# SakodaShintaro/f2-nerf

Measured on AMD Instinct MI355X. Metric: rendered rays/sec (fwd+bwd) at 800x800, higher is better.
Workload: dtype f32; 1 GPU; ngp_fox-like synthetic views 800x800, 128 samples/ray, L=16 F=2 T=2^19, 65536-ray chunks, TRAIN render + loss + backward (optimizer excluded); pixel_order=rows, regime=dense

## Files before the change

f2-nerf_amd/csrc/kernels/hash_grid.hip:

```cpp
#include "hash_grid.hiph"


namespace
{


__global__ __launch_bounds__(F2N_BLOCK) void table_to_f16_kernel(
  const float * __restrict__ in, uint16_t * __restrict__ out, int64_t n)
{
  const int64_t stride = (int64_t)gridDim.x * blockDim.x * 8;
  for (int64_t i = ((int64_t)blockIdx.x * blockDim.x + threadIdx.x) * 8; i < n; i += stride) {
    if (i + 8 <= n) {
      const float4 a = *reinterpret_cast<const float4 *>(in + i);
      const float4 b = *reinterpret_cast<const float4 *>(in + i + 4);
      uint4 o;
      o.x = (uint32_t)__half_as_ushort(__float2half_rn(a.x)) |
            ((uint32_t)__half_as_ushort(__float2half_rn(a.y)) << 16);
      o.y = (uint32_t)__half_as_ushort(__float2half_rn(a.z)) |
            ((uint32_t)__half_as_ushort(__float2half_rn(a.w)) << 16);
      o.z = (uint32_t)__half_as_ushort(__float2half_rn(b.x)) |
            ((uint32_t)__half_as_ushort(__float2half_rn(b.y)) << 16);
      o.w = (uint32_t)__half_as_ushort(__float2half_rn(b.z)) |
            ((uint32_t)__half_as_ushort(__float2half_rn(b.w)) << 16);
      *reinterpret_cast<uint4 *>(out + i) = o;
    } else {
      for (int64_t j = i; j < n; j++) out[j] = __half_as_ushort(__float2half_rn(in[j]));
    }
  }
}


template <int F, bool POW2>
__global__ __launch_bounds__(F2N_BLOCK) void hash_fwd_kernel(
  const float * __restrict__ pts, const uint16_t * __restrict__ table,
  const int32_t * __restrict__ primes, const float * __restrict__ bias,
  const float * __restrict__ mul, float * __restrict__ out, int64_t out_ld_point,
  int64_t out_ld_chan, uint32_t * __restrict__ idx_out, int64_t n, int L, uint32_t T,
  int64_t level_stride)
{
  const int l = blockIdx.y;
  const int64_t p = (int64_t)blockIdx.x * F2N_BLOCK + threadIdx.x;
  if (p >= n) return;
  const LevelParams lp = load_level(primes, bias, mul, l);
  const float x = pts[3 * p + 0], y = pts[3 * p + 1], z = pts[3 * p + 2];
  uint32_t row[8];
  float w[8];
  corner_rows_and_weights<POW2>(x, y, z, lp, T, row, w);
  float acc[F];
  gather_blend<F>(table + level_stride * l, row, w, acc);
  float * o = out + p * out_ld_point + (int64_t)(l * F) * out_ld_chan;
#pragma unroll
  for (int k = 0; k < F; k++) o[k * out_ld_chan] = round_f16(acc[k]);
  if (idx_out) {
    uint32_t * io = idx_out + (p * L + l) * 8;
#pragma unroll
    for (int d = 0; d < 8; d++) io[d] = row[d];
  }
}


template <int F, bool POW2, int SAMPLES>
__global__ __launch_bounds__(F2N_BLOCK) void hash_fwd_raytile_kernel(
  const float * __restrict__ pts, const uint16_t * __restrict__ table,
  const int32_t * __restrict__ primes, const float * __restrict__ bias,
  const float * __restrict__ mul, float * __restrict__ out, int n_rays, int S, uint32_t T,
  int64_t level_stride, int walk, int corner_order)
{
  static_assert(F2N_BLOCK == 256 && SAMPLES % 16 == 0, "4 waves, float4 runs");
  constexpr int RAYS = 64, kPitch = SAMPLES + 4, kPPitch = 3 * SAMPLES + 1;
  __shared__ __attribute__((aligned(16))) float tile[F][RAYS][kPitch];
  __shared__ float ptile[RAYS][kPPitch];
  const int l = blockIdx.y;
  const int tiles_s = S / SAMPLES;
  const int r0 = (int)(blockIdx.x / tiles_s) * RAYS, k0 = (int)(blockIdx.x % tiles_s) * SAMPLES;
  const int lane = threadIdx.x & 63, wave = threadIdx.x >> 6;
  const int64_t n = (int64_t)n_rays * S;
#pragma unroll
  for (int i = 0; i < RAYS * 3 * SAMPLES / 256; i++) {
    const int idx = threadIdx.x + 256 * i;
    const int ray = idx / (3 * SAMPLES), off = idx % (3 * SAMPLES);
    const int r = min(r0 + ray, n_rays - 1);
    ptile[ray][off] = pts[((int64_t)r * S + k0) * 3 + off];
  }
  const LevelParams lp = load_level(primes, bias, mul, l);
  __syncthreads();
  bool along, drifted;
  {
    constexpr int m = SAMPLES / 2;
    auto dist = [&](int ra, int sa, int rb, int sb) {
      const float dx = ptile[ra][3 * sa] - ptile[rb][3 * sb], dy = ptile[ra][3 * sa + 1] - ptile[rb][3 * sb + 1],
                  dz = ptile[ra][3 * sa + 2] - ptile[rb][3 * sb + 2];
      return sqrtf(dx * dx + dy * dy + dz * dz);
    };
    const float e = dist(RAYS - 1, m, 0, m), e1 = dist(1, m, 0, m), sl = dist(0, SAMPLES - 1, 0, 0);
    along = !(e + 8.f * e1 < 2.f * sl);
    if (walk) along = (walk == 2);
    const float apart = fmaxf(e1, fmaxf(dist(RAYS / 2 + 1, m, RAYS / 2, m), dist(RAYS - 1, m, RAYS - 2, m)));
    drifted = apart * (float)(SAMPLES - 1) > 0.35f * sl;
  }
  __shared__ uint16_t order[RAYS * SAMPLES];
  __shared__ uint32_t bin_at[64];
  const bool sorted = !along && (walk == 3 || (walk == 0 && drifted));
  if (sorted) {
    constexpr int kPairs = RAYS * SAMPLES / 256;
    constexpr int mr = RAYS / 2;
    const float ax = ptile[mr][3 * (SAMPLES - 1)] - ptile[mr][0],
                ay = ptile[mr][3 * (SAMPLES - 1) + 1] - ptile[mr][1],
                az = ptile[mr][3 * (SAMPLES - 1) + 2] - ptile[mr][2];
    const float inv = 64.f / fmaxf(ax * ax + ay * ay + az * az, 1e-30f);
    const float ox = ptile[mr][0], oy = ptile[mr][1], oz = ptile[mr][2];
    if (threadIdx.x < 64) bin_at[threadIdx.x] = 0u;
    __syncthreads();
    int my_bin[kPairs];
#pragma unroll
    for (int i = 0; i < kPairs; i++) {
      const int pair = threadIdx.x + 256 * i, ray = pair / SAMPLES, ks = pair % SAMPLES;
      const float d = (ptile[ray][3 * ks] - ox) * ax + (ptile[ray][3 * ks + 1] - oy) * ay +
                      (ptile[ray][3 * ks + 2] - oz) * az;
      my_bin[i] = min(max((int)(d * inv), 0), 63);
      atomicAdd(&bin_at[my_bin[i]], 1u);
    }
    __syncthreads();
    if (wave == 0) {
      const int c = (int)bin_at[lane];
      bin_at[lane] = (uint32_t)(wave_incl_scan_i32(c) - c);
    }
    __syncthreads();
#pragma unroll
    for (int i = 0; i < kPairs; i++)
      order[atomicAdd(&bin_at[my_bin[i]], 1u)] = (uint16_t)(threadIdx.x + 256 * i);
    __syncthreads();
  }
  constexpr int kRaysPerIter = 64 / SAMPLES;
  auto walk_tile = [&](auto paired) {
#pragma unroll
    for (int j = 0; j < SAMPLES / 4; j++) {
      int ks = along ? (lane % SAMPLES) : (j * 4 + wave);
      int ray = along ? ((j * 4 + wave) * kRaysPerIter + lane / SAMPLES) : lane;
      if (sorted) {
        const int pair = order[(j * 4 + wave) * 64 + lane];
        ray = pair / SAMPLES;
        ks = pair % SAMPLES;
      }
      const float x = ptile[ray][3 * ks], y = ptile[ray][3 * ks + 1], z = ptile[ray][3 * ks + 2];
      uint32_t row[8];
      float w[8], acc[F];
      if constexpr (decltype(paired)::value) {
        const uint32_t m = slot_rows_and_weights<POW2>(x, y, z, lp, T, row, w);
        gather_blend_paired<F>(table + level_stride * l, row, m, w, acc);
      } else {
        corner_rows_and_weights<POW2>(x, y, z, lp, T, row, w);
        gather_blend<F>(table + level_stride * l, row, w, acc);
      }
#pragma unroll
      for (int k = 0; k < F; k++) tile[k][ray][ks] = round_f16(acc[k]);
    }
  };
  if (corner_order == 0)
    walk_tile(std::true_type{});
  else
    walk_tile(std::false_type{});
  __syncthreads();
#pragma unroll
  for (int i = 0; i < SAMPLES / 16; i++) {
    const int idx = threadIdx.x + 256 * i;
    const int ray = idx / (SAMPLES / 4), quad = idx % (SAMPLES / 4);
    if (r0 + ray < n_rays) {
#pragma unroll
      for (int k = 0; k < F; k++) {
        const float4 v = *reinterpret_cast<const float4 *>(&tile[k][ray][4 * quad]);
        *reinterpret_cast<float4 *>(
          out + (int64_t)(l * F + k) * n + (int64_t)(r0 + ray) * S + k0 + 4 * quad) = v;
      }
    }
  }
}


template <int F, bool POW2, bool WITH_PTS_GRAD>
__global__ __launch_bounds__(F2N_BLOCK) void hash_bwd_kernel(
  const float * __restrict__ pts, const uint16_t * __restrict__ table,
  const int32_t * __restrict__ primes, const float * __restrict__ bias,
  const float * __restrict__ mul, const float * __restrict__ grad_out, int64_t g_ld_point,
  int64_t g_ld_chan, float * __restrict__ table_grad, float * __restrict__ pts_grad, int64_t n,
  uint32_t T, int64_t level_stride, float grad_scale, float inv_scale)
{
  const int l = blockIdx.y;
  const int64_t p = (int64_t)blockIdx.x * F2N_BLOCK + threadIdx.x;
  if (p >= n) return;
  const LevelParams lp = load_level(primes, bias, mul, l);
  const float x = pts[3 * p + 0], y = pts[3 * p + 1], z = pts[3 * p + 2];
  uint32_t row[8];
  float w[8];
  corner_rows_and_weights<POW2>(x, y, z, lp, T, row, w);

  const float * g = grad_out + p * g_ld_point + (int64_t)(l * F) * g_ld_chan;
  float gk[F];
  bool any = false;
#pragma unroll
  for (int k = 0; k < F; k++) {
    gk[k] = round_f16(g[k * g_ld_chan] * grad_scale);
    any |= (gk[k] != 0.f);
  }
  float * gbase = table_grad + level_stride * l;
  if (any) {
#pragma unroll
    for (int d = 0; d < 8; d++) {
#pragma unroll
      for (int k = 0; k < F; k++) {
        const float c = round_f16(gk[k] * w[d]) * inv_scale;
        atomicAdd(gbase + (int64_t)row[d] * F + k, c);
      }
    }
  }
  if (WITH_PTS_GRAD) {
    using Row = typename RowBits<F>::type;
    const Row * rows = reinterpret_cast<const Row *>(table + level_stride * l);
    float gx = 0.f, gy = 0.f, gz = 0.f;
#pragma unroll
    for (int d = 0; d < 8; d++) {
      float f[F];
      const Row r = rows[row[d]];
      unpack_row<F>(r, f);
#pragma unroll
      for (int k = 0; k < F; k++) {
        const float nrm = f[k] * lp.mul * gk[k];
        const float pos = round_f16(nrm), neg = round_f16(-nrm);
        gx += (d & 4) ? pos : neg;
        gy += (d & 2) ? pos : neg;
        gz += (d & 1) ? pos : neg;
      }
    }
    atomicAdd(pts_grad + 3 * p + 0, gx * inv_scale);
    atomicAdd(pts_grad + 3 * p + 1, gy * inv_scale);
    atomicAdd(pts_grad + 3 * p + 2, gz * inv_scale);
  }
}

constexpr int kSliceFloats = 32768;
constexpr int kSliceBlock = 1024;

template <int F, bool POW2>
__global__ __launch_bounds__(kSliceBlock) void hash_bwd_sliced_kernel(
  const float * __restrict__ pts, const int32_t * __restrict__ primes,
  const float * __restrict__ bias, const float * __restrict__ mul,
  const float * __restrict__ grad_out, int64_t g_ld_point, int64_t g_ld_chan,
  float * __restrict__ table_grad, int64_t n, uint32_t T, int64_t level_stride, float grad_scale,
  float inv_scale, int n_parts)
{
  __shared__ float acc[kSliceFloats];
  constexpr uint32_t kRows = kSliceFloats / F;
  const uint32_t slice = blockIdx.x;
  const int l = blockIdx.y;
  const int part = blockIdx.z;
  const uint32_t row_lo = slice * kRows;

  for (int i = threadIdx.x; i < kSliceFloats; i += kSliceBlock) acc[i] = 0.f;
  __syncthreads();

  const LevelParams lp = load_level(primes, bias, mul, l);
  const int64_t per = (n + n_parts - 1) / n_parts;
  const int64_t p_begin = per * part;
  const int64_t p_end = (p_begin + per < n) ? p_begin + per : n;
  const float * gcol = grad_out + (int64_t)(l * F) * g_ld_chan;

  struct Item
  {
    float x, y, z;
    float g[F];
  };
  auto fetch = [&](int64_t p, Item & it) {
    it.x = pts[3 * p + 0];
    it.y = pts[3 * p + 1];
    it.z = pts[3 * p + 2];
    const float * g = gcol + p * g_ld_point;
#pragma unroll
    for (int k = 0; k < F; k++) it.g[k] = g[k * g_ld_chan];
  };
  auto apply = [&](const Item & it) {
    uint32_t row[8];
    float w[8];
    corner_rows_and_weights<POW2>(it.x, it.y, it.z, lp, T, row, w);
    float gk[F];
#pragma unroll
    for (int k = 0; k < F; k++) gk[k] = round_f16(it.g[k] * grad_scale);
#pragma unroll
    for (int d = 0; d < 8; d++) {
      const uint32_t local = row[d] - row_lo;
      if (local < kRows) {
#pragma unroll
        for (int k = 0; k < F; k++) {
          const float c = round_f16(gk[k] * w[d]);
          if (c != 0.f) atomicAdd(&acc[local * F + k], c);
        }
      }
    }
  };

  int64_t p = p_begin + threadIdx.x;
  if (p < p_end) {
    Item cur, nxt;
    fetch(p, cur);
    for (; p < p_end; p += kSliceBlock) {
      const int64_t pn = (p + kSliceBlock < p_end) ? p + kSliceBlock : p;
      fetch(pn, nxt);
      apply(cur);
      cur = nxt;
    }
  }
  __syncthreads();

  float * gbase = table_grad + level_stride * l + (int64_t)row_lo * F;
  const uint32_t rows_here = (row_lo + kRows <= T) ? kRows : (T > row_lo ? T - row_lo : 0u);
  const int n_flush = (int)rows_here * F;
  for (int i = threadIdx.x; i < n_flush; i += kSliceBlock) {
    const float v = acc[i];
    if (v != 0.f) atomicAdd(gbase + i, v * inv_scale);
  }
}


__global__ __launch_bounds__(F2N_BLOCK) void contract_fwd_kernel(
  const float * __restrict__ pts, float * __restrict__ out, int64_t n)
{
  const int64_t p = (int64_t)blockIdx.x * F2N_BLOCK + threadIdx.x;
  if (p >= n) return;
  float x = pts[3 * p], y = pts[3 * p + 1], z = pts[3 * p + 2];
  contract_point(x, y, z);
  out[3 * p] = x;
  out[3 * p + 1] = y;
  out[3 * p + 2] = z;
}

__global__ __launch_bounds__(F2N_BLOCK) void contract_bwd_kernel(
  const float * __restrict__ pts, const float * __restrict__ dx, float * __restrict__ dp, int64_t n)
{
  const int64_t p = (int64_t)blockIdx.x * F2N_BLOCK + threadIdx.x;
  if (p >= n) return;
  const float x = pts[3 * p], y = pts[3 * p + 1], z = pts[3 * p + 2];
  const float gx = dx[3 * p], gy = dx[3 * p + 1], gz = dx[3 * p + 2];
  const float n2 = fmaf(z, z, fmaf(y, y, x * x));
  const float nrm = sqrtf(n2);
  float ox, oy, oz;
  if (nrm <= 1.f) {
    const float poison = (nrm == 0.f) ? __builtin_nanf("") : 0.f;
    ox = gx + poison;
    oy = gy + poison;
    oz = gz + poison;
  } else {
    const float inv = 1.f / nrm;
    const float a = (2.f - inv) * inv;
    const float da_over_n = (2.f * inv - 2.f) * inv * inv * inv;
    const float pg = fmaf(z, gz, fmaf(y, gy, x * gx));
    const float c = da_over_n * pg;
    ox = fmaf(c, x, a * gx);
    oy = fmaf(c, y, a * gy);
    oz = fmaf(c, z, a * gz);
  }
  dp[3 * p] = ox;
  dp[3 * p + 1] = oy;
  dp[3 * p + 2] = oz;
}

}

extern "C" int f2n_table_to_f16(
  const float * table_f32, uint16_t * table_f16, int64_t n, void * stream)
{
  if (!table_f32 || !table_f16 || n < 0) return F2N_E_INVALID_ARG;
  if (n == 0) return F2N_OK;
  if ((reinterpret_cast<uintptr_t>(table_f32) & 15u) || (reinterpret_cast<uintptr_t>(table_f16) & 15u))
    return F2N_E_INVALID_ARG;
  const int64_t work = (n + 7) / 8;
  const unsigned grid = (unsigned)std::min<int64_t>((work + F2N_BLOCK - 1) / F2N_BLOCK, 256 * 16);
  hipLaunchKernelGGL(
    table_to_f16_kernel, dim3(grid), dim3(F2N_BLOCK), 0, (hipStream_t)stream, table_f32, table_f16,
    n);
  return f2n_launch_status();
}

extern "C" int f2n_hash_fwd(
  const float * pts, const uint16_t * table_f16, const int32_t * primes, const float * bias,
  const float * mul, float * out, int64_t out_ld_point, int64_t out_ld_chan, uint32_t * idx_out,
  int64_t n, int L, int F, uint32_t T, int64_t level_stride, void * stream)
{
  if (!pts || !table_f16 || !primes || !bias || !mul || !out) return F2N_E_INVALID_ARG;
  if (F != 1 && F != 2 && F != 4 && F != 8) return F2N_E_UNSUPPORTED;
  if (!f2n_hash_args_ok(n, L, F, T, level_stride)) return F2N_E_INVALID_ARG;
  if (reinterpret_cast<uintptr_t>(table_f16) % (2u * F)) return F2N_E_INVALID_ARG;
  if (n == 0) return F2N_OK;
  const dim3 grid(f2n_div_up(n, F2N_BLOCK), (unsigned)L), block(F2N_BLOCK);
  hipStream_t s = (hipStream_t)stream;
  f2n_dispatch_field(F, T, [&](auto ff, auto p2) {
    hipLaunchKernelGGL(
      (hash_fwd_kernel<decltype(ff)::value, decltype(p2)::value>), grid, block, 0, s, pts,
      table_f16, primes, bias, mul, out, out_ld_point, out_ld_chan, idx_out, n, L, T, level_stride);
  });
  return f2n_launch_status();
}

extern "C" int f2n_hash_fwd_raytile(
  const float * pts, const uint16_t * table_f16, const int32_t * primes, const float * bias,
  const float * mul, float * out_cm, int n_rays, int S, int L, int F, uint32_t T,
  int64_t level_stride, void * stream)
{
  if (!pts || !table_f16 || !primes || !bias || !mul || !out_cm) return F2N_E_INVALID_ARG;
  if (F != 1 && F != 2 && F != 4 && F != 8) return F2N_E_UNSUPPORTED;
  if (n_rays < 0 || S <= 0) return F2N_E_INVALID_ARG;
  if (S % 16) return F2N_E_UNSUPPORTED;
  const int64_t n = (int64_t)n_rays * S;
  if (!f2n_hash_args_ok(n, L, F, T, level_stride)) return F2N_E_INVALID_ARG;
  if (reinterpret_cast<uintptr_t>(table_f16) % (2u * F)) return F2N_E_INVALID_ARG;
  if (reinterpret_cast<uintptr_t>(out_cm) & 15u) return F2N_E_INVALID_ARG;
  if (n == 0) return F2N_OK;
  const int walk = f2n_get_option(F2N_OPT_RAYTILE_WALK);
  const int corner_order = f2n_get_option(F2N_OPT_GATHER_PAIRED);
  const int want = f2n_get_option(F2N_OPT_RAYTILE);
  const int ts = (want == 16) ? 16 : (S % 32 == 0 ? 32 : 16);
  const int64_t tiles = (int64_t)f2n_div_up(n_rays, 64) * (S / ts);
  if (tiles > 0x7fffffff) return F2N_E_INVALID_ARG;
  const dim3 grid((unsigned)tiles, (unsigned)L), block(F2N_BLOCK);
  hipStream_t s = (hipStream_t)stream;
  f2n_dispatch_field(F, T, [&](auto ff, auto p2) {
    constexpr int FF = decltype(ff)::value;
    constexpr bool P2 = decltype(p2)::value;
    if (ts == 16)
      hipLaunchKernelGGL(
        (hash_fwd_raytile_kernel<FF, P2, 16>), grid, block, 0, s, pts, table_f16, primes, bias, mul,
        out_cm, n_rays, S, T, level_stride, walk, corner_order);
    else
      hipLaunchKernelGGL(
        (hash_fwd_raytile_kernel<FF, P2, 32>), grid, block, 0, s, pts, table_f16, primes, bias, mul,
        out_cm, n_rays, S, T, level_stride, walk, corner_order);
  });
  return f2n_launch_status();
}

extern "C" int f2n_hash_bwd(
  const float * pts, const uint16_t * table_f16, const int32_t * primes, const float * bias,
  const float * mul, const float * grad_out, int64_t g_ld_point, int64_t g_ld_chan,
  float * table_grad, float * pts_grad, int64_t n, int L, int F, uint32_t T, int64_t level_stride,
  float grad_scale, void * stream)
{
  if (!pts || !table_f16 || !primes || !bias || !mul || !grad_out || !table_grad)
    return F2N_E_INVALID_ARG;
  if (F != 1 && F != 2 && F != 4 && F != 8) return F2N_E_UNSUPPORTED;
  if (!f2n_hash_args_ok(n, L, F, T, level_stride)) return F2N_E_INVALID_ARG;
  if (reinterpret_cast<uintptr_t>(table_f16) % (2u * F)) return F2N_E_INVALID_ARG;
  int e = 0;
  const float m = frexpf(grad_scale, &e);
  if (!(grad_scale > 0.f) || m != 0.5f) return F2N_E_INVALID_ARG;
  if (n == 0) return F2N_OK;
  hipStream_t s = (hipStream_t)stream;
  const float inv = 1.f / grad_scale;

  const int64_t rows_per_slice = kSliceFloats / F;
  const int64_t n_slices = ((int64_t)T + rows_per_slice - 1) / rows_per_slice;
  const int force = f2n_get_option(F2N_OPT_HASH_BWD);
  bool sliced = !pts_grad && n_slices <= 64 && n >= 32768;
  if (force && !pts_grad && n_slices <= 1024) sliced = (force == 2);
  if (sliced) {
    int n_parts = 1;
    while ((int64_t)L * n_slices * n_parts < 512 && (n / (n_parts * 2)) >= 65536) n_parts *= 2;
    const dim3 grid((unsigned)n_slices, (unsigned)L, (unsigned)n_parts), block(kSliceBlock);
    f2n_dispatch_field(F, T, [&](auto ff, auto p2) {
      hipLaunchKernelGGL(
        (hash_bwd_sliced_kernel<decltype(ff)::value, decltype(p2)::value>), grid, block, 0, s, pts,
        primes, bias, mul, grad_out, g_ld_point, g_ld_chan, table_grad, n, T, level_stride,
        grad_scale, inv, n_parts);
    });
    return f2n_launch_status();
  }

  if (pts_grad) {
    if (hipMemsetAsync(pts_grad, 0, sizeof(float) * 3 * n, s) != hipSuccess) return F2N_E_LAUNCH;
  }
  const dim3 grid(f2n_div_up(n, F2N_BLOCK), (unsigned)L), block(F2N_BLOCK);
  f2n_dispatch_field(F, T, [&](auto ff, auto p2) {
    constexpr int FF = decltype(ff)::value;
    constexpr bool P2 = decltype(p2)::value;
    if (pts_grad)
      hipLaunchKernelGGL(
        (hash_bwd_kernel<FF, P2, true>), grid, block, 0, s, pts, table_f16, primes, bias, mul,
        grad_out, g_ld_point, g_ld_chan, table_grad, pts_grad, n, T, level_stride, grad_scale, inv);
    else
      hipLaunchKernelGGL(
        (hash_bwd_kernel<FF, P2, false>), grid, block, 0, s, pts, table_f16, primes, bias, mul,
        grad_out, g_ld_point, g_ld_chan, table_grad, pts_grad, n, T, level_stride, grad_scale, inv);
  });
  return f2n_launch_status();
}

extern "C" int f2n_contract_fwd(const float * pts, float * x, int64_t n, void * stream)
{
  if (!pts || !x || n < 0) return F2N_E_INVALID_ARG;
  if (n == 0) return F2N_OK;
  hipLaunchKernelGGL(
    contract_fwd_kernel, dim3(f2n_div_up(n, F2N_BLOCK)), dim3(F2N_BLOCK), 0, (hipStream_t)stream,
    pts, x, n);
  return f2n_launch_status();
}

extern "C" int f2n_contract_bwd(
  const float * pts, const float * dx, float * dpts, int64_t n, void * stream)
{
  if (!pts || !dx || !dpts || n < 0) return F2N_E_INVALID_ARG;
  if (n == 0) return F2N_OK;
  hipLaunchKernelGGL(
    contract_bwd_kernel, dim3(f2n_div_up(n, F2N_BLOCK)), dim3(F2N_BLOCK), 0, (hipStream_t)stream,
    pts, dx, dpts, n);
  return f2n_launch_status();
}
```

include/f2nerf_hip.h:

```cpp
#ifndef F2NERF_HIP_H_
#define F2NERF_HIP_H_

#include <stdint.h>

#ifdef __cplusplus
extern "C" {
#endif

#define F2N_ABI_VERSION 2

#define F2N_OK 0
#define F2N_E_INVALID_ARG (-1)
#define F2N_E_LAUNCH (-2)
#define F2N_E_UNSUPPORTED (-3)

#define F2N_MAX_LEVELS 32

int f2n_abi_version(void);
const char * f2n_status_string(int status);

#define F2N_OPT_SHADE_FWD 0
#define F2N_OPT_SHADE_BWD 1
#define F2N_OPT_SHADE_VARIANT 2
#define F2N_OPT_RAYTILE 3
#define F2N_OPT_HASH_BWD 4
#define F2N_OPT_BWD_COMBINE 5
#define F2N_OPT_RAYTILE_WALK 6
#define F2N_OPT_MARCH 7
#define F2N_OPT_BWD_PHASES 8
#define F2N_OPT_RAY_ORDER 9
#define F2N_OPT_SHADE_BWD_WAVES 10
#define F2N_SHADE_BWD_TWO_WAVES_MIN_SAMPLES (3 << 19)
#define F2N_OPT_SHADE_RAYS 11
#define F2N_OPT_DENSE_LEAN 12
#define F2N_OPT_COUNT 13
#define F2N_OPT2_FIRST 64
#define F2N_OPT_GATHER_PAIRED (F2N_OPT2_FIRST + 0)
#define F2N_OPT2_COUNT 1
int f2n_set_option(int key, int value);
int f2n_get_option(int key);


int f2n_table_to_f16(const float * table_f32, uint16_t * table_f16, int64_t n, void * stream);

int f2n_hash_fwd(
  const float * pts, const uint16_t * table_f16, const int32_t * primes, const float * bias,
  const float * mul, float * out, int64_t out_ld_point, int64_t out_ld_chan, uint32_t * idx_out,
  int64_t n, int L, int F, uint32_t T, int64_t level_stride, void * stream);

int f2n_hash_fwd_raytile(
  const float * pts, const uint16_t * table_f16, const int32_t * primes, const float * bias,
  const float * mul, float * out_cm, int n_rays, int S, int L, int F, uint32_t T,
  int64_t level_stride, void * stream);

int f2n_hash_bwd(
  const float * pts, const uint16_t * table_f16, const int32_t * primes, const float * bias,
  const float * mul, const float * grad_out, int64_t g_ld_point, int64_t g_ld_chan,
  float * table_grad, float * pts_grad, int64_t n, int L, int F, uint32_t T, int64_t level_stride,
  float grad_scale, void * stream);

int64_t f2n_hash_bwd_workspace_bytes(int64_t n, int L, int F, uint32_t T);
int f2n_hash_bwd_set_overflow_counter(uint64_t * device_counter);
int f2n_hash_bwd_binned(
  const float * pts, const int32_t * primes, const float * bias, const float * mul,
  const float * grad_out, int64_t g_ld_point, int64_t g_ld_chan, float * table_grad, int64_t n,
  int L, int F, uint32_t T, int64_t level_stride, float grad_scale, void * workspace,
  int64_t workspace_bytes, void * stream);

int f2n_contract_fwd(const float * pts, float * x, int64_t n, void * stream);
int f2n_contract_bwd(const float * pts, const float * dx, float * dpts, int64_t n, void * stream);

int f2n_hash_rays_grad(
  const float * pts, const float * t, const int32_t * bounds, const float * rays_d,
  const uint16_t * table_f16, const int32_t * primes, const float * bias, const float * mul,
  const float * grad_out, int64_t g_ld_point, int64_t g_ld_chan, float * d_rays_o,
  float * d_rays_d, int n_rays, int L, int F, uint32_t T, int64_t level_stride, float grad_scale,
  void * stream);


int f2n_sh_encode(const float * dirs, float * out, int64_t n, int degree, void * stream);


int f2n_seg_sum_fwd(const float * val, const int32_t * idx, float * sum, int n_rays, void * stream);
int f2n_seg_sum_bwd(const float * dsum, const int32_t * idx, float * dval, int n_rays, void * stream);
int f2n_seg_sum_vec_fwd(
  const float * val, const int32_t * idx, float * sum, int n_rays, int vec, void * stream);
int f2n_seg_sum_vec_bwd(
  const float * dsum, const int32_t * idx, float * dval, int n_rays, int vec, void * stream);
int f2n_seg_scan_fwd(
  const float * val, const int32_t * idx, float * sum, int n_rays, int include_this, void * stream);
int f2n_seg_scan_bwd(
  const float * dsum, const int32_t * idx, float * dval, int n_rays, int include_this,
  void * stream);

int f2n_weight_var_fwd(
  const float * weights, const int32_t * idx, float * out_vars, int n_rays, void * stream);
int f2n_weight_var_bwd(
  const float * weights, const int32_t * idx, const float * dvars, float * dw, int n_rays,
  void * stream);

int f2n_weight_dist_fwd(
  const float * weights, const float * t, const float * dt, const int32_t * idx, float * out,
  int n_rays, void * stream);
int f2n_weight_dist_bwd(
  const float * weights, const float * t, const float * dt, const int32_t * idx,
  const float * d_out, float * dw, int n_rays, void * stream);


int f2n_scatter_idx(
  const int32_t * idx, const int32_t * emb_idx, int32_t * all_emb_idx, int n_rays, void * stream);
int f2n_scatter_add_fwd(
  const float * emb, const int32_t * scatter_idx, const float * to_add, float * sum, int64_t n_all,
  int C, void * stream);
int f2n_scatter_add_bwd(
  const int32_t * scatter_idx, const float * dsum, float * demb, int64_t n_all, int n_emb, int C,
  void * stream);


int f2n_gen_rays(
  const float * poses, int pose_ld, const float * intrinsics, int64_t n_cams,
  const int32_t * cam_idx, const int32_t * ij, int64_t first_pixel, int width, float * rays_o,
  float * rays_d, int64_t n, void * stream);

int64_t f2n_gen_rays_bwd_workspace_floats(int64_t n);
int f2n_gen_rays_bwd(
  const float * intrinsics, int64_t n_cams, const int32_t * ij, int64_t first_pixel, int width,
  const float * d_rays_o, const float * d_rays_d, float * d_poses, int pose_ld, float * workspace,
  int64_t n, void * stream);

int f2n_gen_rays_dist(
  const float * poses, int pose_ld, const float * intrinsics, const float * dist, int64_t n_cams,
  const int32_t * cam_idx, const int32_t * ij, int64_t first_pixel, int width, float * rays_o,
  float * rays_d, int64_t n, void * stream);

int f2n_gen_rays_dist_bwd(
  const float * intrinsics, const float * dist, int64_t n_cams, const int32_t * ij,
  int64_t first_pixel, int width, const float * d_rays_o, const float * d_rays_d, float * d_poses,
  int pose_ld, float * workspace, int64_t n, void * stream);

int64_t f2n_cam_pose_grad_workspace_floats(int64_t n, int64_t n_cams);
int f2n_cam_pose_grad(
  const float * intrinsics, const float * dist, const int32_t * ij, const float * d_rays_o,
  const float * d_rays_d, const int32_t * cam_start, const int32_t * order, float * d_poses,
  int pose_ld, float * workspace, int64_t n, int64_t n_cams, void * stream);

int f2n_pose_compose(
  const float * base, int pose_ld, const float * delta, const int32_t * fixed, float * out,
  int64_t n_cams, void * stream);

int f2n_pose_compose_bwd(
  const float * base, int pose_ld, const float * delta, const int32_t * fixed, const float * d_out,
  float * d_delta, int64_t n_cams, void * stream);

int f2n_project_points(
  const float * points, const float * poses, int pose_ld, const float * intrinsics,
  const float * dist, int64_t n_cams, const int32_t * cam_idx, float * pix, int32_t * valid,
  int64_t n, void * stream);

int f2n_sample_rays(
  const float * rays_o, const float * rays_d, const float * noise, float * pts, float * dirs,
  float * dt, float * t, int32_t * bounds, int n_rays, int S, float step, void * stream);

int f2n_sample_dense(
  const float * rays_o, const float * rays_d, const float * noise, const int32_t * noise_row,
  int noise_affine, float * x, float * dt, float * t, int32_t * bounds, float * ray_dirs,
  int n_rays, int S, float step, void * stream);

int f2n_density_march(
  const float * rays_o, const float * rays_d, const float * noise, const uint16_t * table_f16,
  const int32_t * primes, const float * bias, const float * mul, const float * w0, const float * b0,
  int32_t * kept, int n_rays, int S, float step, int L, int F, uint32_t T, int64_t level_stride,
  float t_thresh, float density_shift, void * stream);

int f2n_density_scan(
  const float * enc_cm, int C, const float * dt, const float * w0, const float * b0, int32_t * kept,
  int n_rays, int S, float t_thresh, float density_shift, void * stream);

int f2n_density_margin(
  const float * logit, const float * dt, int32_t * flag, int n_rays, int S, float density_shift,
  float depth_limit, void * stream);

int f2n_compact_rows_cm(
  const float * src, int64_t n_src, float * dst, int64_t n_dst, int C, const int32_t * bounds,
  int n_rays, int S, void * stream);

int f2n_bounds_from_counts(
  const int32_t * kept, int32_t * bounds, int32_t * total, int n_rays, void * stream);

int f2n_sample_compact(
  const float * rays_o, const float * rays_d, const float * noise, const int32_t * bounds,
  float * pts, float * dirs, float * dt, float * t, int n_rays, int S, float step, void * stream);



int f2n_occ_update(
  const uint16_t * table_f16, const int32_t * primes, const float * bias, const float * mul,
  const float * w0, const float * b0, const float * probe_u, float * density, uint32_t * bits, int G,
  int L, int F, uint32_t T, int64_t level_stride, float density_shift, float threshold, float decay,
  void * stream);

int f2n_occ_lookup(
  const float * pts, int64_t n, const uint32_t * bits, int G, uint8_t * out, void * stream);

int f2n_density_march_occ(
  const float * rays_o, const float * rays_d, const float * noise, const uint16_t * table_f16,
  const int32_t * primes, const float * bias, const float * mul, const float * w0, const float * b0,
  const uint32_t * bits, int G, int32_t * kept, int32_t * len, int n_rays, int S, float step, int L,
  int F, uint32_t T, int64_t level_stride, float t_thresh, float density_shift, void * stream);

int f2n_sample_compact_occ(
  const float * rays_o, const float * rays_d, const float * noise, const int32_t * bounds,
  const int32_t * len, const uint32_t * bits, int G, float * pts, float * dirs, float * dt,
  float * t, int n_rays, int S, float step, void * stream);


int f2n_ray_keys(const float * rays_d, int32_t * keys, int n, void * stream);

int f2n_ray_permute(
  const int64_t * order, int n, int S, const float * rays_o, const float * rays_d,
  const int32_t * emb_idx, const float * bg, const float * noise, int32_t * perm, float * rays_o_p,
  float * rays_d_p, int32_t * emb_idx_p, float * bg_p, float * noise_p, int32_t * inv,
  void * stream);

int f2n_gather_rows(
  const float * src, float * dst, const int32_t * map, int n, int row_floats, void * stream);

int f2n_gather_segments(
  const float * src, const int32_t * src_bounds, float * dst, const int32_t * dst_bounds,
  const int32_t * map, int n_rays, void * stream);

int f2n_counts_through(
  const int32_t * bounds, const int32_t * map, int32_t * counts, int n_rays, void * stream);


int f2n_composite_fwd(
  const float * logit, int64_t logit_ld, const float * rgb, const float * dt, const float * t,
  const int32_t * bounds, const float * bg, float * colors, float * depths, float * weights,
  float * last_trans, int n_rays, float density_shift, float t_shift, void * stream);

int f2n_composite_bwd(
  const float * logit, int64_t logit_ld, const float * rgb, const float * dt, const float * t,
  const int32_t * bounds, const float * bg, const float * weights, const float * last_trans,
  const float * d_colors, const float * d_depths, const float * d_weights, float * d_logit,
  float * d_rgb, int n_rays, float density_shift, float t_shift, void * stream);


int f2n_shade_fwd(
  const float * enc_cm, int C, const float * dirs, const int32_t * sample_img, const float * w_h,
  const float * b_h, const float * w1, const float * b1, const float * w2, const float * b2,
  const float * app_emb, float * logit, float * rgb, float * pre_cm, int64_t n, void * stream);

int f2n_shade_bwd(
  const float * enc_cm, int C, const float * dirs, const int32_t * sample_img, const float * w_h,
  const float * b_h, const float * w1, const float * b1, const float * w2, const float * b2,
  const float * app_emb, const float * d_logit, const float * d_rgb, float * d_enc_cm,
  float * g_w_h, float * g_b_h, float * g_w1, float * g_b1, float * g_w2, float * g_b2,
  float * g_app_emb, const float * pre_cm, int64_t n, void * stream);

int f2n_shade_fwd_rays(
  const float * enc_cm, int C, const float * dirs, const int32_t * ray_img, const float * w_h,
  const float * b_h, const float * w1, const float * b1, const float * w2, const float * b2,
  const float * app_emb, float * logit, float * rgb, int n_rays, int S, void * stream);

int f2n_shade_bwd_rays(
  const float * enc_cm, int C, const float * dirs, const int32_t * ray_img, const float * w_h,
  const float * b_h, const float * w1, const float * b1, const float * w2, const float * b2,
  const float * app_emb, const float * d_logit, const float * d_rgb, float * d_enc_cm,
  float * g_w_h, float * g_b_h, float * g_w1, float * g_b1, float * g_w2, float * g_b2,
  float * g_app_emb, int n_rays, int S, void * stream);

int f2n_shade_fwd_raydirs(
  const float * enc_cm, int C, const float * ray_dirs, const int32_t * ray_img, const float * w_h,
  const float * b_h, const float * w1, const float * b1, const float * w2, const float * b2,
  const float * app_emb, float * logit, float * rgb, int n_rays, int S, void * stream);

int f2n_shade_bwd_raydirs(
  const float * enc_cm, int C, const float * ray_dirs, const int32_t * ray_img, const float * w_h,
  const float * b_h, const float * w1, const float * b1, const float * w2, const float * b2,
  const float * app_emb, const float * d_logit, const float * d_rgb, float * d_enc_cm,
  float * g_w_h, float * g_b_h, float * g_w1, float * g_b1, float * g_w2, float * g_b2,
  float * g_app_emb, int n_rays, int S, void * stream);


int f2n_render_rays(
  const float * rays_o, const float * rays_d, const float * noise ,
  const uint16_t * table, const int32_t * primes, const float * bias, const float * mul,
  const float * w_h, const float * b_h, const float * w1, const float * b1,
  const float * w2, const float * b2,
  const float * app_emb, const int32_t * ray_img ,
  const uint32_t * occ_bits , int G,
  const float * bg, float * colors, float * depths, float * last_trans,
  int32_t * kept, int32_t * len ,
  int n_rays, int S, float step, int L, int F, uint32_t T, int64_t level_stride,
  float t_thresh, float density_shift, float t_shift, void * stream);

int64_t f2n_render_rays_state_bytes(int n_rays);
int f2n_render_rays_head(
  const float * rays_o, const float * rays_d, const float * noise ,
  const uint16_t * table, const int32_t * primes, const float * bias, const float * mul,
  const float * w_h, const float * b_h, const float * w1, const float * b1,
  const float * w2, const float * b2,
  const float * app_emb, const int32_t * ray_img ,
  const uint32_t * occ_bits , int G,
  const float * bg, float * colors, float * depths, float * last_trans,
  int32_t * kept, int32_t * len ,
  int n_rays, int S, float step, int L, int F, uint32_t T, int64_t level_stride,
  float t_thresh, float density_shift, float t_shift, int n_head, void * state, void * stream);
int f2n_render_rays_tail(
  const float * rays_o, const float * rays_d, const float * noise ,
  const uint16_t * table, const int32_t * primes, const float * bias, const float * mul,
  const float * w_h, const float * b_h, const float * w1, const float * b1,
  const float * w2, const float * b2,
  const float * app_emb, const int32_t * ray_img ,
  const uint32_t * occ_bits , int G,
  const float * bg, float * colors, float * depths, float * last_trans,
  int32_t * kept, int32_t * len ,
  int n_rays, int S, float step, int L, int F, uint32_t T, int64_t level_stride,
  float t_thresh, float density_shift, float t_shift, int n_head, const void * state,
  void * stream);


int f2n_adam_step(
  float * param, const float * grad, float * exp_avg, float * exp_avg_sq, uint16_t * shadow_f16,
  int64_t n, float lr, float beta1, float beta2, float eps, float weight_decay, int step,
  void * stream);

int64_t f2n_loss_workspace_floats(int n_rays);
int f2n_loss_fwd(
  const float * colors, const float * gt, const float * var, int n_rays, float var_weight,
  float * d_colors, float * d_var, float * partial, float * out4, void * stream);


int f2n_perturb_poses(
  const float * pose, int pose_ld, const float * noise, float sigma_pos_x, float sigma_pos_y,
  float sigma_pos_z, float sigma_rot_x, float sigma_rot_y, float sigma_rot_z, float * poses, int P,
  void * stream);

int f2n_pose_scores(
  const float * colors, const float * image, const int32_t * ij, float * loss, float * weights,
  double * workspace, int P, int K, int h, int w, void * stream);

int f2n_average_pose(
  const float * poses, const float * weights, float * pose_out, int P, void * stream);

#ifdef __cplusplus
}
#endif

#endif
```

Measured before the change: 12.88 million rays/s.

## Process groups of coarse hash levels per raytile block to reuse staged points

Adds a raytile forward kernel in which each block handles a contiguous group of levels instead of one. The block stages the tile's points, walk choice and depth order once, keeps each lane's points in registers, and loops over levels with double-buffered LDS output tiles. A default grouping merges coarse levels into one block and keeps fine levels single or paired, which cuts repeated point loads and sorting work and shrinks the grid. The cost is fewer blocks, less parallelism for the coarse levels, and more LDS per block.

```diff
diff --git a/f2-nerf_amd/csrc/kernels/hash_grid.hip b/f2-nerf_amd/csrc/kernels/hash_grid.hip
--- a/f2-nerf_amd/csrc/kernels/hash_grid.hip
+++ b/f2-nerf_amd/csrc/kernels/hash_grid.hip
@@ -59,6 +59,62 @@
 }
 
 
+
+template <int SAMPLES>
+__device__ __forceinline__ void raytile_walk_choice(
+  const float * ptile, int walk, bool & along, bool & sorted)
+{
+  constexpr int RAYS = 64, kPPitch = 3 * SAMPLES + 1;
+  constexpr int m = SAMPLES / 2;
+  auto dist = [&](int ra, int sa, int rb, int sb) {
+    const float * a = ptile + ra * kPPitch + 3 * sa, * b = ptile + rb * kPPitch + 3 * sb;
+    const float dx = a[0] - b[0], dy = a[1] - b[1], dz = a[2] - b[2];
+    return sqrtf(dx * dx + dy * dy + dz * dz);
+  };
+  const float e = dist(RAYS - 1, m, 0, m), e1 = dist(1, m, 0, m), sl = dist(0, SAMPLES - 1, 0, 0);
+  along = !(e + 8.f * e1 < 2.f * sl);
+  if (walk) along = (walk == 2);
+  const float apart =
+    fmaxf(e1, fmaxf(dist(RAYS / 2 + 1, m, RAYS / 2, m), dist(RAYS - 1, m, RAYS - 2, m)));
+  const bool drifted = apart * (float)(SAMPLES - 1) > 0.35f * sl;
+  sorted = !along && (walk == 3 || (walk == 0 && drifted));
+}
+
+template <int SAMPLES>
+__device__ __forceinline__ void raytile_depth_order(
+  const float * ptile, uint16_t * order, uint32_t * bin_at)
+{
+  constexpr int RAYS = 64, kPPitch = 3 * SAMPLES + 1;
+  constexpr int kPairs = RAYS * SAMPLES / 256;
+  const int lane = threadIdx.x & 63, wave = threadIdx.x >> 6;
+  const float * mid = ptile + (RAYS / 2) * kPPitch;
+  const float ax = mid[3 * (SAMPLES - 1)] - mid[0], ay = mid[3 * (SAMPLES - 1) + 1] - mid[1],
+              az = mid[3 * (SAMPLES - 1) + 2] - mid[2];
+  const float inv = 64.f / fmaxf(ax * ax + ay * ay + az * az, 1e-30f);
+  const float ox = mid[0], oy = mid[1], oz = mid[2];
+  if (threadIdx.x < 64) bin_at[threadIdx.x] = 0u;
+  __syncthreads();
+  int my_bin[kPairs];
+#pragma unroll
+  for (int i = 0; i < kPairs; i++) {
+    const int pair = threadIdx.x + 256 * i, ray = pair / SAMPLES, ks = pair % SAMPLES;
+    const float * p = ptile + ray * kPPitch + 3 * ks;
+    const float d = (p[0] - ox) * ax + (p[1] - oy) * ay + (p[2] - oz) * az;
+    my_bin[i] = min(max((int)(d * inv), 0), 63);
+    atomicAdd(&bin_at[my_bin[i]], 1u);
+  }
+  __syncthreads();
+  if (wave == 0) {
+    const int c = (int)bin_at[lane];
+    bin_at[lane] = (uint32_t)(wave_incl_scan_i32(c) - c);
+  }
+  __syncthreads();
+#pragma unroll
+  for (int i = 0; i < kPairs; i++)
+    order[atomicAdd(&bin_at[my_bin[i]], 1u)] = (uint16_t)(threadIdx.x + 256 * i);
+  __syncthreads();
+}
+
 template <int F, bool POW2, int SAMPLES>
 __global__ __launch_bounds__(F2N_BLOCK) void hash_fwd_raytile_kernel(
   const float * __restrict__ pts, const uint16_t * __restrict__ table,
@@ -84,53 +140,11 @@
   }
   const LevelParams lp = load_level(primes, bias, mul, l);
   __syncthreads();
-  bool along, drifted;
-  {
-    constexpr int m = SAMPLES / 2;
-    auto dist = [&](int ra, int sa, int rb, int sb) {
-      const float dx = ptile[ra][3 * sa] - ptile[rb][3 * sb], dy = ptile[ra][3 * sa + 1] - ptile[rb][3 * sb + 1],
-                  dz = ptile[ra][3 * sa + 2] - ptile[rb][3 * sb + 2];
-      return sqrtf(dx * dx + dy * dy + dz * dz);
-    };
-    const float e = dist(RAYS - 1, m, 0, m), e1 = dist(1, m, 0, m), sl = dist(0, SAMPLES - 1, 0, 0);
-    along = !(e + 8.f * e1 < 2.f * sl);
-    if (walk) along = (walk == 2);
-    const float apart = fmaxf(e1, fmaxf(dist(RAYS / 2 + 1, m, RAYS / 2, m), dist(RAYS - 1, m, RAYS - 2, m)));
-    drifted = apart * (float)(SAMPLES - 1) > 0.35f * sl;
-  }
   __shared__ uint16_t order[RAYS * SAMPLES];
   __shared__ uint32_t bin_at[64];
-  const bool sorted = !along && (walk == 3 || (walk == 0 && drifted));
-  if (sorted) {
-    constexpr int kPairs = RAYS * SAMPLES / 256;
-    constexpr int mr = RAYS / 2;
-    const float ax = ptile[mr][3 * (SAMPLES - 1)] - ptile[mr][0],
-                ay = ptile[mr][3 * (SAMPLES - 1) + 1] - ptile[mr][1],
-                az = ptile[mr][3 * (SAMPLES - 1) + 2] - ptile[mr][2];
-    const float inv = 64.f / fmaxf(ax * ax + ay * ay + az * az, 1e-30f);
-    const float ox = ptile[mr][0], oy = ptile[mr][1], oz = ptile[mr][2];
-    if (threadIdx.x < 64) bin_at[threadIdx.x] = 0u;
-    __syncthreads();
-    int my_bin[kPairs];
-#pragma unroll
-    for (int i = 0; i < kPairs; i++) {
-      const int pair = threadIdx.x + 256 * i, ray = pair / SAMPLES, ks = pair % SAMPLES;
-      const float d = (ptile[ray][3 * ks] - ox) * ax + (ptile[ray][3 * ks + 1] - oy) * ay +
-                      (ptile[ray][3 * ks + 2] - oz) * az;
-      my_bin[i] = min(max((int)(d * inv), 0), 63);
-      atomicAdd(&bin_at[my_bin[i]], 1u);
-    }
-    __syncthreads();
-    if (wave == 0) {
-      const int c = (int)bin_at[lane];
-      bin_at[lane] = (uint32_t)(wave_incl_scan_i32(c) - c);
-    }
-    __syncthreads();
-#pragma unroll
-    for (int i = 0; i < kPairs; i++)
-      order[atomicAdd(&bin_at[my_bin[i]], 1u)] = (uint16_t)(threadIdx.x + 256 * i);
-    __syncthreads();
-  }
+  bool along, sorted;
+  raytile_walk_choice<SAMPLES>(&ptile[0][0], walk, along, sorted);
+  if (sorted) raytile_depth_order<SAMPLES>(&ptile[0][0], order, bin_at);
   constexpr int kRaysPerIter = 64 / SAMPLES;
   auto walk_tile = [&](auto paired) {
 #pragma unroll
@@ -174,6 +188,107 @@
       }
     }
   }
+}
+
+template <int F, bool POW2, int SAMPLES>
+__global__ __launch_bounds__(F2N_BLOCK) void hash_fwd_raytile_kernel_groups(
+  const float * __restrict__ pts, const uint16_t * __restrict__ table,
+  const int32_t * __restrict__ primes, const float * __restrict__ bias,
+  const float * __restrict__ mul, float * __restrict__ out, int n_rays, int S, int L, uint32_t T,
+  int64_t level_stride, int walk, int corner_order, uint32_t group_starts)
+{
+  static_assert(F2N_BLOCK == 256 && SAMPLES % 16 == 0, "4 waves, float4 runs");
+  constexpr int RAYS = 64, kPitch = SAMPLES + 4, kPPitch = 3 * SAMPLES + 1;
+  constexpr int kPairs = SAMPLES / 4;
+  constexpr int kTile = F * RAYS * kPitch, kChan = RAYS * kPitch;
+  constexpr int kPts = RAYS * kPPitch, kOrder = RAYS * SAMPLES / 2, kBins = 64;
+  constexpr int kSecond = (kTile > kPts + kOrder + kBins) ? kTile : (kPts + kOrder + kBins);
+  __shared__ __attribute__((aligned(16))) float lds[kTile + kSecond];
+  float * const ptile = lds + kTile;
+  uint16_t * const order = reinterpret_cast<uint16_t *>(ptile + kPts);
+  uint32_t * const bin_at = reinterpret_cast<uint32_t *>(ptile + kPts + kOrder);
+
+  uint32_t starts = group_starts | 1u;
+  for (int g = blockIdx.y; g > 0; g--) starts &= starts - 1u;
+  const int l0 = __builtin_ctz(starts);
+  starts &= starts - 1u;
+  const int l1 = starts ? __builtin_ctz(starts) : L;
+
+  const int tiles_s = S / SAMPLES;
+  const int r0 = (int)(blockIdx.x / tiles_s) * RAYS, k0 = (int)(blockIdx.x % tiles_s) * SAMPLES;
+  const int lane = threadIdx.x & 63, wave = threadIdx.x >> 6;
+  const int64_t n = (int64_t)n_rays * S;
+#pragma unroll
+  for (int i = 0; i < RAYS * 3 * SAMPLES / 256; i++) {
+    const int idx = threadIdx.x + 256 * i;
+    const int ray = idx / (3 * SAMPLES), off = idx % (3 * SAMPLES);
+    const int r = min(r0 + ray, n_rays - 1);
+    ptile[ray * kPPitch + off] = pts[((int64_t)r * S + k0) * 3 + off];
+  }
+  __syncthreads();
+  bool along, sorted;
+  raytile_walk_choice<SAMPLES>(ptile, walk, along, sorted);
+  if (sorted) raytile_depth_order<SAMPLES>(ptile, order, bin_at);
+  constexpr int kRaysPerIter = 64 / SAMPLES;
+  float px[kPairs], py[kPairs], pz[kPairs];
+  int at[kPairs];
+#pragma unroll
+  for (int j = 0; j < kPairs; j++) {
+    int ks = along ? (lane % SAMPLES) : (j * 4 + wave);
+    int ray = along ? ((j * 4 + wave) * kRaysPerIter + lane / SAMPLES) : lane;
+    if (sorted) {
+      const int pair = order[(j * 4 + wave) * 64 + lane];
+      ray = pair / SAMPLES;
+      ks = pair % SAMPLES;
+    }
+    const float * p = ptile + ray * kPPitch + 3 * ks;
+    px[j] = p[0];
+    py[j] = p[1];
+    pz[j] = p[2];
+    at[j] = ray * kPitch + ks;
+  }
+  auto run_levels = [&](auto paired) {
+    float * tl = lds;
+#pragma unroll 1
+    for (int l = l0; l < l1; l++) {
+      const LevelParams lp = load_level(primes, bias, mul, l);
+      const uint16_t * level_base = table + level_stride * l;
+#pragma unroll
+      for (int j = 0; j < kPairs; j++) {
+        uint32_t row[8];
+        float w[8], acc[F];
+        if constexpr (decltype(paired)::value) {
+          const uint32_t m = slot_rows_and_weights<POW2>(px[j], py[j], pz[j], lp, T, row, w);
+          gather_blend_paired<F>(level_base, row, m, w, acc);
+        } else {
+          corner_rows_and_weights<POW2>(px[j], py[j], pz[j], lp, T, row, w);
+          gather_blend<F>(level_base, row, w, acc);
+        }
+#pragma unroll
+        for (int k = 0; k < F; k++) tl[k * kChan + at[j]] = round_f16(acc[k]);
+      }
+      __syncthreads();
+#pragma unroll
+      for (int i = 0; i < SAMPLES / 16; i++) {
+        const int idx = threadIdx.x + 256 * i;
+        const int ray = idx / (SAMPLES / 4), quad = idx % (SAMPLES / 4);
+        if (r0 + ray < n_rays) {
+#pragma unroll
+          for (int k = 0; k < F; k++) {
+            const float4 v =
+              *reinterpret_cast<const float4 *>(&tl[k * kChan + ray * kPitch + 4 * quad]);
+            *reinterpret_cast<float4 *>(
+              out + (int64_t)(l * F + k) * n + (int64_t)(r0 + ray) * S + k0 + 4 * quad) = v;
+          }
+        }
+      }
+      tl = (tl == lds) ? lds + kTile : lds;
+    }
+  };
+  if (corner_order == 0)
+    run_levels(std::true_type{});
+  else
+    run_levels(std::false_type{});
 }
 
 
@@ -399,32 +514,65 @@
   return f2n_launch_status();
 }
 
-extern "C" int f2n_hash_fwd_raytile(
+constexpr int64_t kFewTiles = 1024;
+
+static uint32_t raytile_default_groups(int L, int64_t tiles)
+{
+  const bool few = tiles < kFewTiles;
+  uint32_t starts = 1u;
+  int first_fine = -1;
+  bool middle_open = false;
+  for (int l = 1; l < L; l++) {
+    if (3 * l >= 2 * (L - 1)) {
+      if (first_fine < 0) first_fine = l;
+      if (few || (l - first_fine) % 2 == 0) starts |= 1u << l;
+    } else if (few && 5 * l >= 2 * (L - 1) && !middle_open) {
+      starts |= 1u << l;
+      middle_open = true;
+    }
+  }
+  return starts;
+}
+
+static int raytile_args_status(
   const float * pts, const uint16_t * table_f16, const int32_t * primes, const float * bias,
   const float * mul, float * out_cm, int n_rays, int S, int L, int F, uint32_t T,
-  int64_t level_stride, void * stream)
+  int64_t level_stride)
 {
   if (!pts || !table_f16 || !primes || !bias || !mul || !out_cm) return F2N_E_INVALID_ARG;
   if (F != 1 && F != 2 && F != 4 && F != 8) return F2N_E_UNSUPPORTED;
   if (n_rays < 0 || S <= 0) return F2N_E_INVALID_ARG;
   if (S % 16) return F2N_E_UNSUPPORTED;
-  const int64_t n = (int64_t)n_rays * S;
-  if (!f2n_hash_args_ok(n, L, F, T, level_stride)) return F2N_E_INVALID_ARG;
+  if (!f2n_hash_args_ok((int64_t)n_rays * S, L, F, T, level_stride)) return F2N_E_INVALID_ARG;
   if (reinterpret_cast<uintptr_t>(table_f16) % (2u * F)) return F2N_E_INVALID_ARG;
   if (reinterpret_cast<uintptr_t>(out_cm) & 15u) return F2N_E_INVALID_ARG;
-  if (n == 0) return F2N_OK;
+  return F2N_OK;
+}
+
+static int raytile_launch(
+  const float * pts, const uint16_t * table_f16, const int32_t * primes, const float * bias,
+  const float * mul, float * out_cm, int n_rays, int S, int L, int F, uint32_t T,
+  int64_t level_stride, int ts, uint32_t group_starts, void * stream)
+{
   const int walk = f2n_get_option(F2N_OPT_RAYTILE_WALK);
   const int corner_order = f2n_get_option(F2N_OPT_GATHER_PAIRED);
-  const int want = f2n_get_option(F2N_OPT_RAYTILE);
-  const int ts = (want == 16) ? 16 : (S % 32 == 0 ? 32 : 16);
   const int64_t tiles = (int64_t)f2n_div_up(n_rays, 64) * (S / ts);
   if (tiles > 0x7fffffff) return F2N_E_INVALID_ARG;
-  const dim3 grid((unsigned)tiles, (unsigned)L), block(F2N_BLOCK);
+  const unsigned rows = group_starts ? (unsigned)__builtin_popcount(group_starts) : (unsigned)L;
+  const dim3 grid((unsigned)tiles, rows), block(F2N_BLOCK);
   hipStream_t s = (hipStream_t)stream;
   f2n_dispatch_field(F, T, [&](auto ff, auto p2) {
     constexpr int FF = decltype(ff)::value;
     constexpr bool P2 = decltype(p2)::value;
-    if (ts == 16)
+    if (group_starts && ts == 16)
+      hipLaunchKernelGGL(
+        (hash_fwd_raytile_kernel_groups<FF, P2, 16>), grid, block, 0, s, pts, table_f16, primes,
+        bias, mul, out_cm, n_rays, S, L, T, level_stride, walk, corner_order, group_starts);
+    else if (group_starts)
+      hipLaunchKernelGGL(
+        (hash_fwd_raytile_kernel_groups<FF, P2, 32>), grid, block, 0, s, pts, table_f16, primes,
+        bias, mul, out_cm, n_rays, S, L, T, level_stride, walk, corner_order, group_starts);
+    else if (ts == 16)
       hipLaunchKernelGGL(
         (hash_fwd_raytile_kernel<FF, P2, 16>), grid, block, 0, s, pts, table_f16, primes, bias, mul,
         out_cm, n_rays, S, T, level_stride, walk, corner_order);
@@ -434,6 +582,46 @@
         out_cm, n_rays, S, T, level_stride, walk, corner_order);
   });
   return f2n_launch_status();
+}
+
+extern "C" int64_t f2n_hash_raytile_default_groups(int L, int64_t tiles)
+{
+  if (L < 1 || tiles < 0) return F2N_E_INVALID_ARG;
+  if (L > 32) return F2N_E_UNSUPPORTED;
+  return (int64_t)raytile_default_groups(L, tiles);
+}
+
+extern "C" int f2n_hash_fwd_raytile(
+  const float * pts, const uint16_t * table_f16, const int32_t * primes, const float * bias,
+  const float * mul, float * out_cm, int n_rays, int S, int L, int F, uint32_t T,
+  int64_t level_stride, void * stream)
+{
+  const int st = raytile_args_status(
+    pts, table_f16, primes, bias, mul, out_cm, n_rays, S, L, F, T, level_stride);
+  if (st != F2N_OK) return st;
+  if (n_rays == 0) return F2N_OK;
+  const int want = f2n_get_option(F2N_OPT_RAYTILE);
+  const int ts = (want == 16) ? 16 : (S % 32 == 0 ? 32 : 16);
+  return raytile_launch(
+    pts, table_f16, primes, bias, mul, out_cm, n_rays, S, L, F, T, level_stride, ts,
+    want ? 0u : raytile_default_groups(L, (int64_t)f2n_div_up(n_rays, 64) * (S / ts)), stream);
+}
+
+extern "C" int f2n_hash_fwd_raytile_groups(
+  const float * pts, const uint16_t * table_f16, const int32_t * primes, const float * bias,
+  const float * mul, float * out_cm, int n_rays, int S, int L, int F, uint32_t T,
+  int64_t level_stride, uint32_t group_starts, void * stream)
+{
+  if (!pts || !table_f16 || !primes || !bias || !mul || !out_cm) return F2N_E_INVALID_ARG;
+  if (L > 32) return F2N_E_UNSUPPORTED;
+  const int st = raytile_args_status(
+    pts, table_f16, primes, bias, mul, out_cm, n_rays, S, L, F, T, level_stride);
+  if (st != F2N_OK) return st;
+  if (L < 32 && (group_starts >> L)) return F2N_E_INVALID_ARG;
+  if (n_rays == 0) return F2N_OK;
+  return raytile_launch(
+    pts, table_f16, primes, bias, mul, out_cm, n_rays, S, L, F, T, level_stride,
+    S % 32 == 0 ? 32 : 16, group_starts | 1u, stream);
 }
 
 extern "C" int f2n_hash_bwd(
diff --git a/include/f2nerf_hip.h b/include/f2nerf_hip.h
--- a/include/f2nerf_hip.h
+++ b/include/f2nerf_hip.h
@@ -52,6 +52,13 @@
   const float * pts, const uint16_t * table_f16, const int32_t * primes, const float * bias,
   const float * mul, float * out_cm, int n_rays, int S, int L, int F, uint32_t T,
   int64_t level_stride, void * stream);
+
+int f2n_hash_fwd_raytile_groups(
+  const float * pts, const uint16_t * table_f16, const int32_t * primes, const float * bias,
+  const float * mul, float * out_cm, int n_rays, int S, int L, int F, uint32_t T,
+  int64_t level_stride, uint32_t group_starts, void * stream);
+
+int64_t f2n_hash_raytile_default_groups(int L, int64_t tiles);
 
 int f2n_hash_bwd(
   const float * pts, const uint16_t * table_f16, const int32_t * primes, const float * bias,
```

After: 13.22 million rays/s, median of 6. +2.7%, better.
